# llsurreal919/Reduce-Complexity-for-intra-coding-of-VVC

Measured on AMD Instinct MI355X. Metric: CTUs/sec (All-Intra, QP32), higher is better.
Workload: dtype int16/int32 samples+coefficients, fp64 RD cost

## Files before the change

reduce-complexity-for-intra-coding-of-vvc_amd/csrc/vvcx_dev.h:

```cpp
#pragma once
#include <stdint.h>

#ifndef VXD_NW
#define VXD_NW 4
#endif
#define VXD_NT (VXD_NW * 64)
#ifndef VXD_BUF
#define VXD_BUF 256
#endif
#ifndef VXD_WPE
#define VXD_WPE 5
#endif
#define VXD_MAXD 12
#define VXD_NUM_CTX 291

struct VxUnit {
  uint64_t ss;
  int16_t  x, y;
  uint8_t  lw, lh;
  uint8_t  qt, mt, bt, depth;
  uint8_t  dir, mrl, cbf, mts;
  uint16_t tag;
};

// ... 154 lines not shown
#define VXD_OFF_SLOTS   ((VXD_OFF_CTX + (VXD_MAXD + VXD_NW + 1) * 2 * VXD_CTXSNAP + 255) & ~255)
#define VXD_SLOT_ELEMS  (2 * 4096)
#define VXD_OFF_TMP     (VXD_OFF_SLOTS + VXD_NW * 2 * VXD_SLOT_ELEMS * 2)
struct VxCacheEnt { uint64_t ss; uint8_t kind , dir, mrl, cbf, depth, mts; uint16_t gen ; };
#define VXD_CACHE_ENTRIES (32 * 32 * 5 * 5)
#define VXD_CACHE_DIM   1152
#define VXD_OFF_ORG     (VXD_OFF_TMP + VXD_NW * 2048 * 4)
#define VXD_OFF_LM      (VXD_OFF_ORG + 4096 * 2)
#define VXD_DQ_WAVE     8192
#define VXD_OFF_DQ      ((VXD_OFF_LM + (1024 + 128) * 2 + 255) & ~255)
#define VXD_POOL_ELEMS      32768
#define VXD_POOL_NODE_BYTES (128 * 1024)
#define VXD_POOL_ITEMS      64
struct VxRbItem { double cost; uint64_t dist, bits; int32_t cbf, sum0, test, wave; };
#define VXD_OFF_POOL    ((VXD_OFF_DQ + VXD_NW * VXD_DQ_WAVE + 255) & ~255)
#define VXD_OFF_POOL_COEF  (VXD_OFF_POOL + VXD_POOL_ELEMS * 2)
#define VXD_OFF_POOL_NODES (VXD_OFF_POOL_COEF + VXD_POOL_ELEMS * 2)
#define VXD_OFF_POOL_REC   (VXD_OFF_POOL_NODES + VXD_POOL_NODE_BYTES)
#define VXD_ISP_WAVE    14336
#define VXD_OFF_ISP     ((VXD_OFF_POOL_REC + 2 * VXD_POOL_ITEMS * (int) sizeof(VxRbItem) + 255) & ~255)
#define VXD_OFF_ISP_BEST (VXD_OFF_ISP + VXD_NW * VXD_ISP_WAVE * 2)
#define VXD_OFF_JCCR    ((VXD_OFF_ISP_BEST + 2 * 4096 * 2 + 255) & ~255)
#define VXD_JCCR_WAVE   (6 * 1024 * 2)
#define VXD_OFF_CACHE   ((VXD_OFF_JCCR + VXD_NW * VXD_JCCR_WAVE + 255) & ~255)
#define VXD_OFF_CACHE_LEV (VXD_OFF_CACHE + VXD_CACHE_ENTRIES * (int) sizeof(VxCacheEnt))
#define VXD_OFF_META    (VXD_OFF_CACHE_LEV + VXD_CACHE_DIM * VXD_CACHE_DIM * 2)
#define VXD_SCRATCH_BYTES (VXD_OFF_META + 256)
```

reduce-complexity-for-intra-coding-of-vvc_amd/csrc/vvcx_kernel.hip:

```cpp
#include <hip/hip_runtime.h>
#include <stdint.h>
#define VX_QUAL static __device__ const
#include "vvcx_tables.h"
#include "vvcx_ctu_syntax_tables.h"
#include "vvcx_dev.h"
#include "vvcx_mip_dev.h"

#define NT VXD_NT
#if (VXD_NW & (VXD_NW - 1)) == 0
#define VTX ((threadIdx.x + ((((unsigned) blockIdx.x * 0x9E3779B1u) >> 30) << 6)) & (unsigned) (VXD_NT - 1))
#else
__device__ inline unsigned vtx_rotated()
{
  const unsigned t = threadIdx.x + ((((unsigned) blockIdx.x * 0x9E3779B1u) >> 24) % VXD_NW << 6);
  return t >= VXD_NT ? t - VXD_NT : t;
}
#define VTX (vtx_rotated())
#endif
#define NW VXD_NW
#define MAXD VXD_MAXD
#define BUF VXD_BUF
#define NCTX VXD_NUM_CTX
static_assert(VXD_NUM_CTX == VX_NUM_CTX, "vvcx_dev.h and the generated tables disagree on the number of context models");
#define MAX_DOUBLE 1.7e+308
// ... 69 lines not shown
  int8_t testIsp, ispSlot, ispPrev, ispNT, ispBestMode, ispBestSplit, ispNOrig, ispNList, ispRegN, ispHadN, skipMts2, ispBreak, ispStop[2], ispNumTotal[2], ispCandIdx[2], ispNTested[2];
  uint8_t ispTMode[16], ispTInfo[16], ispList[28], ispReg[16], ispHad[24], ispWinMode, ispWinSplit, ispWinTucbf;
  double ispTCost[16], ispBestRd, ispCurBest, noIspCost;
  unsigned long long ispWinDist, ispWinBits;
  alignas(4) int8_t ispPartsOf[2][68]; int8_t ispFirst[2][2];
  uint8_t inv0[16], rdSrc[24];
};

#define BIN_FRAC(st_, bin_) L.t.bin_frac[(unsigned) (st_) ^ ((0u - (unsigned) (bin_)) & 255u)]
struct Tables {
  uint32_t bin_frac[256];
  int32_t  qscale[12], iqscale[12];
  int16_t  ang[32], inv_ang[32];
  int8_t   gauss[128], cubic[128];
  uint8_t  last_prefix[8], mode_shift[8];
  uint8_t  ctx_rate[NCTX + 2], gorice_pars[32], gorice_pos0[96], rice_len[128], group_idx[64], mode_num[36], intra_thr[8];
  uint8_t  cg_scan[84], grp_scan[228];
  uint8_t  cg_inv[84], grp_inv[228];
};

#define DQ_ABS_SINGLE 64
#define RC_LIST 320
#define DQ_TAB_INTS (21 * 6 + 3 * 12 * 2 + 4)
struct WaveRc { uint16_t binbuf[RC_LIST]; uint8_t binsort[RC_LIST + 8]; };
struct alignas(16) WaveScratch { WaveRc rc; };
struct WaveMem {
  WaveScratch ws;
  alignas(16) int32_t tmp[BUF];
  alignas(16) int16_t slot[2 * BUF];
};
#define CI_CUR 0
#define CI_W(w) (1 + (w))
struct Lds {
  Tables t;
  Ctx ctxs[1 + NW];
  alignas(16) int16_t org[BUF];
  alignas(16) WaveMem wm[NW];
  int acc[NW][4][2];
  int16_t refs[4][2][140];
  uint8_t flags[72]; int8_t src_unit[72];
  int cache_gen, cur_stream;
  int dq_abs[DQ_ABS_SINGLE + NW];
  Frame fr[MAXD];
  int op, op_a, op_b, op_c, op_d, op_ch;
  int pre_copy_d;
  int nx, ny, nw, nh, nd;
  Cand cand[64]; union { double cand_cost[64]; IspRes isp_res[NW]; }; int n_cand;
// ... 429 lines not shown
  rc_serial<WR>(cb, coeff, w, h, is_chroma, scan, pre, zo);
}
__device__ inline int lane_prefix(unsigned long long m)
{
  return (int) __builtin_amdgcn_mbcnt_hi((unsigned) (m >> 32), __builtin_amdgcn_mbcnt_lo((unsigned) m, 0u));
}
__device__ inline int prefix3(int v, int &total)
{
  const unsigned long long b0 = __ballot(v & 1), b1 = __ballot(v & 2), b2 = __ballot(v & 4);
  total = __popcll(b0) + 2 * __popcll(b1) + 4 * __popcll(b2);
  return lane_prefix(b0) + 2 * lane_prefix(b1) + 4 * lane_prefix(b2);
}
__device__ inline int rem_abs_len(unsigned bins, unsigned rice)
{
  const unsigned thr = 5u << rice;
  if (bins < thr) return (int) ((bins >> rice) + 1 + rice);
  const unsigned maxPrefix = 32 - 5 - 15;
  unsigned prefix = 0, suffix, code = (bins >> rice) - 5;
  if (code >= ((1u << maxPrefix) - 1)) { prefix = maxPrefix; suffix = 15; }
  else { while (code > ((2u << prefix) - 2)) prefix++; suffix = prefix + rice + 1; }
  return (int) (5 + prefix + suffix);
}
#define RC_MAXJ 5
__device__ __noinline__ void rc_chain(int ci, int wv, int nb, int lane, unsigned long long &bits)
{
  nb = uni(nb); ci = uni(ci); wv = uni(wv);
  Ctx *c = &L.ctxs[ci]; const uint16_t *bb = L.wm[wv].ws.rc.binbuf; uint8_t *sorted = L.wm[wv].ws.rc.binsort;
  int ctxv[RC_MAXJ]; unsigned binv[RC_MAXJ]; unsigned long long rem[RC_MAXJ];
#pragma unroll
  for (int j = 0; j < RC_MAXJ; j++) {
    const int k = lane + 64 * j;
    const unsigned e = (j * 64 < nb && k < nb) ? bb[k] : 0xffffu;
    ctxv[j] = e == 0xffffu ? -1 : (int) (e >> 1); binv[j] = e & 1;
    rem[j] = j * 64 < nb ? __ballot(ctxv[j] >= 0) : 0ull;
  }
  int segpos = 0;
  for (;;) {
    int nseg = 0, myctx = 0, mystart = 0, mylen = 0;
    for (;;) {
      int v = -1;
#pragma unroll
      for (int j = 0; j < RC_MAXJ; j++) if (v < 0 && rem[j]) v = __builtin_amdgcn_readlane(ctxv[j], __ffsll(rem[j]) - 1);
      if (v < 0) break;
      const int start = segpos;
#pragma unroll
      for (int j = 0; j < RC_MAXJ; j++) if (rem[j]) {
        const unsigned long long m = __ballot(ctxv[j] == v);
        if (ctxv[j] == v) sorted[segpos + lane_prefix(m)] = (uint8_t) binv[j];
        segpos += __popcll(m); rem[j] &= ~m;
      }
      if (lane == nseg) { myctx = v; mystart = start; mylen = segpos - start; }
      if (++nseg == 64) break;
    }
    if (nseg == 0) break;
    wave_sync();
    if (lane < nseg) {
      unsigned a = c->s0[myctx], b = c->s1[myctx];
      const int rate = L.t.ctx_rate[myctx];
      const int r0 = 2 + ((rate >> 2) & 3), r1 = 3 + r0 + (rate & 3);
      const unsigned i0 = (0x7fffu >> r0) & 0x7FE0u, i1 = (0x7fffu >> r1) & 0x7FFEu;
      unsigned acc = 0, pend = 0, nxt = sorted[mystart];
      for (int k = 0; k < mylen; k++) {
        const unsigned bin = nxt;
        nxt = sorted[mystart + k + 1];
        acc += pend;
        pend = BIN_FRAC((a + b) >> 8, bin);
        a -= (a >> r0) & 0x7FE0u; b -= (b >> r1) & 0x7FFEu;
        if (bin) { a += i0; b += i1; }
      }
      c->s0[myctx] = (uint16_t) a; c->s1[myctx] = (uint16_t) b;
      bits += acc + pend;
    }
    wave_sync();
    if (nseg < 64) break;
  }
}
template <bool SMALL>
__device__ __noinline__ void residual_coding_wave(Cab &cb, int lev_off, const int16_t *coeff_g, int w, int h, int is_chroma, int lane, int zo = 0)
{
  coeff_g = uni_p(coeff_g); lev_off = uni(lev_off);
  zo = uni(zo);
  const int dq = uni((int) (L.par.tools & TOOL_DEPQUANT)) != 0;
  int dqx = 0, dqy = 0;
  const long long q0 = STAMP();
  const int16_t *coeff = SMALL ? L.wm[uni(VTX >> 6)].slot + BUF + uni(lev_off) : coeff_g;
  const RcPre pre = rc_prepass_wave<SMALL>(lev_off, coeff_g, w, h, lane);
  const int last = uni(pre.last);
  if (lane == 0) L.rc_last[uni(VTX >> 6)] = last;
  if (last < 0) return;
  w = uni(w); h = uni(h); is_chroma = uni(is_chroma);
  const ScanGeo geo = scan_geo(w, h);
  const long long q1 = STAMP();
  long long qe = 0, qc = 0;
  const int wv = uni(VTX >> 6);
  uint16_t *bb = L.wm[wv].ws.rc.binbuf; uint8_t *sorted = L.wm[wv].ws.rc.binsort;
  const int lcg = geo.lcg, cgSize = 1 << lcg;
  const int zw = imin(32, w), zh = imin(32, h), wg = geo.wg, hg = geo.hg;
  const unsigned long long sigGroups = pre.sig_groups, sigRaster = pre.sig_raster;
  unsigned long long mybits = 0;
  int nb;
  {
    const int l2w = ilog2i(w), l2h = ilog2i(h);
    int offx = 0, offy = 0, shx, shy;
    if (is_chroma) { shx = imin(2, w >> 3); shy = imin(2, h >> 3); }
    else { offx = L.t.last_prefix[l2w]; offy = L.t.last_prefix[l2h]; shx = (l2w + 1) >> 2; shy = (l2h + 1) >> 2; }
    const int blk = scan_blk(geo, last);
    const int posY = blk >> ilog2i(w), posX = blk & (w - 1);
    const int gx = uni(L.t.group_idx[posX]), gy = uni(L.t.group_idx[posY]);
    const int maxX = L.t.group_idx[((zo && w == 32) ? 16 : zw) - 1], maxY = L.t.group_idx[((zo && h == 32) ? 16 : zh) - 1];
    const int nX = gx + (gx < maxX), nY = gy + (gy < maxY);
    if (lane < nX) bb[lane] = (uint16_t) (((VX_CTX_LastX[is_chroma] + offx + (lane >> shx)) << 1) | (lane < gx));
    if (lane < nY) bb[nX + lane] = (uint16_t) (((VX_CTX_LastY[is_chroma] + offy + (lane >> shy)) << 1) | (lane < gy));
    if (lane == 0) mybits += (unsigned long long) ((gx > 3 ? (gx - 2) >> 1 : 0) + (gy > 3 ? (gy - 2) >> 1 : 0)) << 15;
    nb = nX + nY;
  }
  const int sigBase = VX_CTX_SigFlag[is_chroma], g1Base = VX_CTX_GtxFlag[is_chroma + 2], g2Base = VX_CTX_GtxFlag[is_chroma], parBase = VX_CTX_ParFlag[is_chroma];
  const int grpBase = VX_CTX_SigCoeffGroup[is_chroma];
  int regBins = (((zo && w == 32) ? 16 : zw) * ((zo && h == 32) ? 16 : zh) * 28) >> 4;
// ... 56 lines not shown
      const int sigLower = (cgY + 1) < hg ? (int) ((sigRaster >> (cgPos + wg)) & 1) : 0;
      bb[o++] = (uint16_t) (((grpBase + (sigRight | sigLower)) << 1) | (int) ((sigGroups >> sub) & 1));
    }
    int ep = (coded && a) ? 1 : 0;
    if (ctxMode) {
      if (sigCoded) bb[o++] = (uint16_t) (((VX_CTX_SigFlag[is_chroma + 2 * imax(0, qstate - 1)] + sigofs) << 1) | (a != 0));
      if (a) {
        bb[o++] = (uint16_t) (((g1Base + goff) << 1) | (a > 1));
        if (a > 1) {
          bb[o++] = (uint16_t) (((parBase + goff) << 1) | ((a - 2) & 1));
          bb[o++] = (uint16_t) (((g2Base + goff) << 1) | (((a - 2) >> 1) != 0));
          if (a >= 4) ep += rem_abs_len((unsigned) (a - 4) >> 1, L.t.gorice_pars[imax(imin(sumPlain - 20, 31), 0)]);
        }
      }
    } else if (coded) {
      const int sumAll = imin(sumPlain, 31);
      const unsigned rice = L.t.gorice_pars[sumAll], pos0 = L.t.gorice_pos0[imax(0, qstate - 1) * 32 + sumAll];
      ep += rem_abs_len(a == 0 ? pos0 : (unsigned) a <= pos0 ? (unsigned) a - 1 : (unsigned) a, rice);
    }
    mybits += (unsigned long long) ep << 15;
    regBins -= used; nb += tot;
    wave_sync();
    const long long e1 = STAMP();
    rc_chain(cb.ci, wv, nb, lane, mybits);
    nb = 0;
    qe += e1 - e0; qc += STAMP() - e1;
  }
  const long long q3 = STAMP();
  const unsigned long long tot = wave_sum_u64(mybits);
  if (lane == 0) cb.bits += tot;
  if (VVCX_STAMP && VTX == 0) { PROF(32) += (unsigned long long) (q1 - q0); PROF(34) += (unsigned long long) qe; PROF(35) += (unsigned long long) qc; PROF(36) += (unsigned long long) (STAMP() - q3); PROF(37) += 1; }
}

#include "vvcx_depquant_dev.h"
#include "vvcx_lfnst_dev.h"

__device__ int implicit_split(const VxParams &p, Frame &f, int ch)
{
  if (f.impl_checked) return f.impl_split;
  int split = SPLIT_NONE;
  const int blIn = f.x < p.pic_w && (f.y + f.h - 1) < p.pic_h;
  const int trIn = (f.x + f.w - 1) < p.pic_w && f.y < p.pic_h;
  const int maxBt = p.max_bt_size[ch], minQt = p.min_qt[ch];
  const int btAllowed = f.w <= maxBt && f.h <= maxBt;
  const int qtAllowed = f.w > minQt && f.h > minQt && f.bt == 0;
  if (!blIn && !trIn && qtAllowed) split = SPLIT_QT;
  else if (!blIn && btAllowed) split = SPLIT_BH;
// ... 1352 lines not shown
    }
    if (uni(cbf)) residual_coding_wave<SMALL>(cb, 0, lev, w, h, 0, lane, mts > 1);
    if (lane == 0) cost = rd_cost(p, cb.bits, sse);
    if (VVCX_STAMP && VTX == 0) { const long long tb3 = STAMP(); PROF(28) += (unsigned long long) (tb1 - tb0); PROF(29) += (unsigned long long) (tb2 - tb1); PROF(31) += (unsigned long long) (tb3 - tb2); }
    cost = lane0_d(cost);
    if (cost < mbest) {
      mbest = cost;
      if (lane == 0) { L.rd_cost[c] = cost; L.rd_dist[c] = sse; L.rd_bits[c] = cb.bits; L.rd_cbf[c] = (uint8_t) cbf; L.rd_mts[c] = (uint8_t) mts; L.rd_wave[c] = (uint8_t) wave; }
    }
    if (cost < wbest) {
      wbest = cost;
      if (lane == 0) { L.wave_best[wave] = c; L.wave_slot[wave] = SMALL ? 1 : cur; }
      if (SMALL) { int16_t *pr = slot_rec(scratch, P, wave, 1), *pl = slot_lev(scratch, P, wave, 1); for (int i = lane; i < P; i += 64) { pr[i] = rec[i]; pl[i] = lev[i]; } }
      else cur ^= 1;
      { uint32_t *d = (uint32_t *) ctx_ptr(scratch, CTX_START, MAXD + wave, 0); const uint32_t *s = (const uint32_t *) &L.ctxs[CI_W(wave)]; for (int i = lane; i < NCTX; i += 64) d[i] = s[i]; }
    }
    wave_sync();
    }
  }
  if (lane == 0) L.mts_evals[wave] = nmts;
}
template <bool SMALL> __device__ __noinline__ void stage_b_loop_dct2(uint8_t *scratch, int wave, int lane, int w, int h) { stage_b_loop<SMALL, false>(L.par, scratch, wave, lane, w, h); }
template <bool SMALL> __device__ __noinline__ void stage_b_loop_mts(const VxParams &p_, uint8_t *scratch, int wave, int lane, int w, int h) { stage_b_loop<SMALL, true>(L.par, scratch, wave, lane, w, h); (void) p_; }
template <bool SMALL>
__device__ void dq_trellis_phase(uint8_t *scratch, int n, int P, int total, int w, int h, int zo, int wave, int lane, int lfnst = 0, int item0 = 0, int abs0 = 0, int wave_shift = 0)
{
  int16_t *poolCoef = (int16_t *) (scratch + VXD_OFF_POOL_COEF) + (size_t) item0 * P; uint8_t *poolNodes = scratch + VXD_OFF_POOL_NODES + (size_t) item0 * 4 * total;
  const int ipw = imin(16, (int) sizeof(WaveMem) / (240 + 2 * total));
  for (int i0 = ((wave + NW - wave_shift) % NW) * ipw; i0 < n; i0 += NW * ipw)
    wave_depquant_batch<2>(imin(ipw, n - i0), poolCoef + (size_t) i0 * P, P, poolNodes + (size_t) i0 * 4 * total, 4 * total, wave, abs0 + i0,
                        CI_CUR, 0, VX_CTX_QtCbf[0], 0u, w, h, 0, zo, lfnst, lane);
}
template <bool SMALL>
__device__ __noinline__ void stage_b_rounds(uint8_t *scratch, int wave, int lane, int w, int h)
{
  scratch = uni_p(scratch); wave = uni(wave); w = uni(w); h = uni(h);
  const VxParams &p = L.par;
  const int P = w * h, bd = uni(p.bit_depth), total = imin(32, w) * imin(32, h);
  const int mtsOk = mts_allowed(p, w, h);
  const int lfOn = uni((int) (p.tools & TOOL_LFNST)) != 0, psLf = lfOn ? uni((int) L.ps_lfnst) : 0, psMts = lfOn ? uni((int) L.ps_mts) : 0, psGrp = uni((int) L.ps_grp);
  const int pruneOk = mtsOk && !lfOn;
  const int tsOn = lfOn && !psLf && !psMts && ts_allowed(p, w, h);
  int16_t *poolPred = (int16_t *) (scratch + VXD_OFF_POOL), *poolCoef = (int16_t *) (scratch + VXD_OFF_POOL_COEF);
  VxRbItem *recA = (VxRbItem *) (scratch + VXD_OFF_POOL_REC), *recB = recA + VXD_POOL_ITEMS;
  const int capItems = imin(VXD_POOL_ITEMS, imin(VXD_POOL_ELEMS / P, VXD_POOL_NODE_BYTES / (4 * total)));
  const int capCand = imin(16, pruneOk ? imax(1, capItems / 3) : capItems);
// ... 24 lines not shown
        for (int e = lane; e < P; e += 64) { const int py = e >> ilog2i(w), px = e & (w - 1); rec[e] = (int16_t) pred_sample(top, left, w, h, px, py, ip, mode, 1, bd, dcv); }
      }
      wave_sync();
      for (int e = lane; e < P; e += 64) poolPred[(size_t) i * P + e] = rec[e];
      unsigned long long sse; int cbf, sum0 = 0;
      const int mtsC = psMts ? pass_mts_idx(psGrp, mode) : 0;
      if (mtsC) wave_code_block_mts<SMALL>(org, rec, lev, wave_tmp(scratch, imin(w, 32) * h, wave), w, h, bd, p.qp_tr, mtsC, lane, sse, cbf, -2);
      else wave_code_block<SMALL, true>(org, 0, 0, rec, lev, wave_tmp(scratch, imin(w, 32) * h, wave), w, h, bd, p.qp_tr, lane, sse, cbf, -2, &sum0, 0, 0, 0, psLf, psLf ? lfnst_mode(mip ? PLANAR : mode, w, h) : 0);
      for (int e = lane; e < P; e += 64) poolCoef[(size_t) i * P + e] = lev[e];
      if (lane == 0) { recA[i].sum0 = sum0; recA[i].test = 0; recB[i].sum0 = sum0; }
      if (specGen) {
        wave_code_block_mts<SMALL>(org, rec, lev, wave_tmp(scratch, imin(w, 32) * h, wave), w, h, bd, p.qp_tr, 2, lane, sse, cbf, -2);
        for (int e = lane; e < P; e += 64) poolCoef[(size_t) (nA + i) * P + e] = lev[e];
      }
      if (specGen2) {
        wave_code_block<SMALL>(org, 0, 0, rec, lev, wave_tmp(scratch, imin(w, 32) * h, wave), w, h, bd, p.qp_tr, lane, sse, cbf, -2, nullptr, 0, 0, 0, 2, lfnst_mode(mip ? PLANAR : mode, w, h));
        for (int e = lane; e < P; e += 64) poolCoef[(size_t) (nA + i) * P + e] = lev[e];
      }
    }
    __threadfence_block();
    __syncthreads();
    const long long q1 = STAMP();
    if (!specUse) dq_trellis_phase<SMALL>(scratch, nA, P, total, w, h, psMts, wave, lane, psLf);
    if (specGen) dq_trellis_phase<SMALL>(scratch, nA, P, total, w, h, 1, wave, lane, 0, nA, 32, 1);
    if (specGen2) dq_trellis_phase<SMALL>(scratch, nA, P, total, w, h, 0, wave, lane, 2, nA, 32, 1);
    if (tsEarly && wave >= 2) {
      for (int i = wave - 2; i < nA; i += 2) {
        const int sa = wave_ts_fwd(org, poolPred + (size_t) i * P, poolCoef + (size_t) (48 + i) * P, w, h, bd, lane);
        if (lane == 0) L.rb_pairs[i] = (uint8_t) ((double) sa <= (double) recB[i].sum0);
      }
      __threadfence_block();
      wave_sync();
      int cnt = 0, mine = -1;
      for (int i = wave - 2; i < nA; i += 2) if (L.rb_pairs[i]) { if (cnt == lane) mine = i; cnt++; }
      if (mine >= 0) L.dq_abs[48 + mine] = ts_rdoq_lane(poolCoef + (size_t) (48 + mine) * P, w, h, bd, p.qp_tr);
    }
    __threadfence_block();
    __syncthreads();
    const long long q2 = STAMP();
    if (specGen || specGen2) { if ((int) VTX < nA) L.spec_abs[VTX] = L.dq_abs[32 + VTX]; if (VTX == 0) { L.spec_n = (int8_t) nA; L.spec_kind = (int8_t) (specGen ? 1 : 2); } }
    else if (VTX == 0) L.spec_n = 0;
    for (int i = wave; i < nA; i += NW) {
      const int c = c0 + i, mode = uni(L.rd[c].mode), mrl = uni(L.rd[c].mrl);
      int16_t *rec = SMALL ? L.wm[wave].slot : slot_rec(scratch, P, wave, cur), *lev = SMALL ? L.wm[wave].slot + BUF : slot_lev(scratch, P, wave, cur);
      const int mtsC = psMts ? pass_mts_idx(psGrp, mode) : 0;
      const int src = specUse ? (specKind == 2 ? i : uni((int) L.rd_src[c])) : i;
      for (int e = lane; e < P; e += 64) { rec[e] = poolPred[(size_t) src * P + e]; lev[e] = poolCoef[(size_t) (specUse ? specN + src : i) * P + e]; }
      wave_sync();
// ... 125 lines not shown
        { uint32_t *d = (uint32_t *) &L.ctxs[CI_W(wave)]; const uint32_t *s = (const uint32_t *) &L.ctxs[CI_CUR]; for (int e = lane; e < NCTX; e += 64) d[e] = s[e]; }
        wave_sync();
        double cost = 0;
        Cab cb; cb.ci = CI_W(wave); cb.bits = 0;
        if (lane == 0) { enc_intra_luma_pred_mode(cb, L.ny, mode, mrl); enc_bin(cb, 1u, VX_CTX_QtCbf[0]); enc_tu_mts(cb, w, h, mts); }
        residual_coding_wave<SMALL>(cb, 0, lev, w, h, 0, lane, 1);
        if (lane == 0) { cost = rd_cost(p, cb.bits, sse); recB[j].cost = cost; recB[j].dist = sse; recB[j].bits = cb.bits; }
        cost = lane0_d(cost);
        if (cost < wbest || (cost == wbest && c * 8 + k < wkey)) {
          wbest = cost; wkey = c * 8 + k;
          if (lane == 0) { L.wave_best[wave] = c; L.wave_slot[wave] = SMALL ? 1 : cur; }
          if (SMALL) { int16_t *pr = slot_rec(scratch, P, wave, 1), *pl = slot_lev(scratch, P, wave, 1); for (int e = lane; e < P; e += 64) { pr[e] = rec[e]; pl[e] = lev[e]; } }
          else cur ^= 1;
          { uint32_t *d = (uint32_t *) ctx_ptr(scratch, CTX_START, MAXD + wave, 0); const uint32_t *s = (const uint32_t *) &L.ctxs[CI_W(wave)]; for (int e = lane; e < NCTX; e += 64) d[e] = s[e]; }
        }
        wave_sync();
      }
      __threadfence_block();
      __syncthreads();
    }
    if (VVCX_STAMP && VTX == 0) { PROF(38) += (unsigned long long) (q1 - q0); PROF(39) += (unsigned long long) (q2 - q1); PROF(40) += (unsigned long long) (q3 - q2); PROF(41) += (unsigned long long) (STAMP() - q3); PROF(44) += 1; PROF(45) += (unsigned long long) nA; }
#ifdef VVCX_STAMP_PASS
    if (VTX == 0) { const int kind = psMts ? 3 + psGrp : psLf; PROF(16 + kind) += 1; PROF(23 + kind) += (unsigned long long) (q2 - q1); }
#endif
    if ((int) VTX < nA) {
      const int i = VTX, c = c0 + i;
      double bc = recA[i].cost; uint64_t bd_ = recA[i].dist, bb = recA[i].bits; int bcbf = recA[i].cbf, bm = 0, bw = recA[i].wave;
      for (int j = 0; j < nB; j++) if ((pi_[j] >> 3) == i) { const double v = recB[j].cost; if (v < bc) { bc = v; bd_ = recB[j].dist; bb = recB[j].bits; bcbf = 1; bm = (pi_[j] & 7) + 1; bw = recB[j].wave; } }
      if (lfOn) { bm = recA[i].sum0 >> 8; L.rd_lfl[c] = (uint8_t) (recA[i].sum0 & 3); }
      L.rd_cost[c] = bc; L.rd_dist[c] = bd_; L.rd_bits[c] = bb; L.rd_cbf[c] = (uint8_t) bcbf; L.rd_mts[c] = (uint8_t) bm; L.rd_wave[c] = (uint8_t) bw;
    }
    __syncthreads();
  }
  if (lane == 0) L.mts_evals[wave] = nmts;
}
__device__ __noinline__ void op_stage_b(const VxParams &p_, uint8_t *scratch)
{
  scratch = uni_p(scratch);
  const VxParams &p = L.par; (void) p_;
  const int wave = uni(VTX >> 6), lane = VTX & 63;
  const int w = uni(L.nw), h = uni(L.nh);
  if (uni(p.tools & TOOL_DEPQUANT)) { if (w * h <= BUF) stage_b_rounds<true>(scratch, wave, lane, w, h); else stage_b_rounds<false>(scratch, wave, lane, w, h); }
  else if (uni(p.tools & TOOL_MTS)) { if (w * h <= BUF) stage_b_loop_mts<true>(p, scratch, wave, lane, w, h); else stage_b_loop_mts<false>(p, scratch, wave, lane, w, h); }
  else if (w * h <= BUF) stage_b_loop_dct2<true>(scratch, wave, lane, w, h); else stage_b_loop_dct2<false>(scratch, wave, lane, w, h);
  __threadfence_block();
  __syncthreads();
// ... 115 lines not shown
__device__ inline int ict_mode(int sign, int mask) { const int m = mask == 1 ? 3 : mask == 2 ? 1 : 2; return sign ? -m : m; }
__device__ inline int ict_fwd(int b, int r, int mode, long long &err)
{
  int v, eb, er;
  switch (mode) {
    case  1: v = (4 * b + 2 * r) / 5; eb = b - v; er = r - (v >> 1); break;
    case -1: v = (4 * b - 2 * r) / 5; eb = b - v; er = r - (-v >> 1); break;
    case  2: v = (b + r) / 2; eb = b - v; er = r - v; break;
    case -2: v = (b - r) / 2; eb = b - v; er = r + v; break;
    case  3: v = (4 * r + 2 * b) / 5; eb = b - (v >> 1); er = r - v; break;
    default: v = (4 * r - 2 * b) / 5; eb = b - (-v >> 1); er = r - v; break;
  }
  err += (long long) eb * eb + (long long) er * er;
  return v;
}
__device__ inline int ict_inv(int c, int mode, int k)
{
  const int am = mode < 0 ? -mode : mode, sc = mode < 0 ? -c : c;
  if (am == 3) return k == 1 ? c : (sc >> 1);
  return k == 0 ? c : (am == 1 ? (sc >> 1) : sc);
}
__device__ inline long long wave_sum_i64(long long v) { return (long long) wave_sum_u64((unsigned long long) v); }

template <bool SMALL>
__device__ __noinline__ void chroma_rd_rounds(uint8_t *scratch, int wave, int lane, int w, int h)
{
  scratch = uni_p(scratch); wave = uni(wave); w = uni(w); h = uni(h);
  const VxParams &p = L.par;
  const int P = w * h, bd = uni(p.bit_depth), total = imin(32, w) * imin(32, h);
  const int16_t *lmin = lm_in_buf(scratch, 2 * P);
  const int16_t *org = org_tile(scratch, 2 * P);
  int16_t *poolPred = (int16_t *) (scratch + VXD_OFF_POOL), *poolCoef = (int16_t *) (scratch + VXD_OFF_POOL_COEF); uint8_t *poolNodes = scratch + VXD_OFF_POOL_NODES;
  if (lane == 0) L.wave_best[wave] = -1;
  dq_build_tables(1);
  double wbest = MAX_DOUBLE;
  int cur = 0;
  const int n_rd = uni(L.n_rd);
  const int psLf = (uni((int) (p.tools & TOOL_LFNST)) && w >= 4 && h >= 4) ? uni((int) L.ps_lfnst) : 0;
  const int jccrOn = uni((int) (p.tools & TOOL_JCCR)) != 0;
  const int cadj = P > 4 ? uni(L.lmcs_cadj) : 0;
  int njoint = 0;
#define CHROMA_LFMODE(c_) (psLf ? lfnst_mode((uni((int) L.rd[c_].mode) >= LM_CHROMA && uni((int) L.rd[c_].mode) <= MDLM_T) ? uni(L.colm) : uni((int) L.rd[c_].mrl), w, h) : 0)
  for (int c = wave; c < n_rd; c += NW) {
    const int fm = uni(L.rd[c].mrl), lfm = CHROMA_LFMODE(c);
    int16_t *recb = SMALL ? L.wm[wave].slot : slot_rec(scratch, 2 * P, wave, cur), *levb = SMALL ? L.wm[wave].slot + BUF : slot_lev(scratch, 2 * P, wave, cur);
    for (int k = 0; k < 2; k++) {
// ... 5 lines not shown
      wave_code_block<SMALL>(org, k * P, k * P, rec, lev, wave_tmp(scratch, imin(w, 32) * h, wave), w, h, bd, p.qp_tr_c[k], lane, sse, cbf, -2, nullptr, k + 1, CI_CUR, 0, psLf, lfm, 0, -1, cadj);
      for (int e = lane; e < P; e += 64) poolCoef[(size_t) (2 * c + k) * P + e] = lev[e];
      wave_sync();
    }
  }
  __threadfence_block();
  __syncthreads();
  {
    const int ipw = imin(16, (int) sizeof(WaveMem) / (240 + 2 * total));
    for (int i0 = wave * ipw; i0 < n_rd; i0 += NW * ipw)
      wave_depquant_batch<2>(imin(ipw, n_rd - i0), poolCoef + (size_t) (2 * i0) * P, 2 * P, poolNodes + (size_t) (2 * i0) * 4 * total, 8 * total, wave, i0,
                          CI_CUR, 0, VX_CTX_QtCbf[1], 0u, w, h, 1, 0, psLf, lane);
  }
  __threadfence_block();
  __syncthreads();
  const bool crBatch = 4 * (240 + 2 * total) <= (int) (sizeof(WaveScratch) + sizeof(int32_t) * BUF);
  for (int c0 = 0; c0 < n_rd; c0 += NW) {
    const int c = c0 + wave; const bool have = c < n_rd;
    const int cm = have ? uni(L.rd[c].mode) : 0;
    const int lfm = have ? CHROMA_LFMODE(c) : 0;
    int16_t *recb = SMALL ? L.wm[wave].slot : slot_rec(scratch, 2 * P, wave, cur), *levb = SMALL ? L.wm[wave].slot + BUF : slot_lev(scratch, 2 * P, wave, cur);
    unsigned long long dist = 0; int cbfs[2] = { 0, 0 };
    double compCost = 0; int jccr = 0;
    if (have) {
      { uint32_t *d = (uint32_t *) &L.ctxs[CI_W(wave)]; const uint32_t *s_ = (const uint32_t *) &L.ctxs[CI_CUR]; for (int e = lane; e < NCTX; e += 64) d[e] = s_[e]; }
      for (int e = lane; e < P; e += 64) { recb[e] = poolPred[(size_t) (2 * c) * P + e]; levb[e] = poolCoef[(size_t) (2 * c) * P + e]; }
      wave_sync();
      cbfs[0] = uni(L.dq_abs[c]) > 0;
      unsigned long long sse; int cbf2;
      wave_code_block<SMALL>(org, 0, 0, recb, levb, wave_tmp(scratch, imin(w, 32) * h, wave), w, h, bd, p.qp_tr_c[0], lane, sse, cbf2, cbfs[0], nullptr, 1, CI_W(wave), 0, psLf, lfm, 0, -1, cadj);
      dist += (unsigned long long) (p.dist_weight[0] * (double) sse);
      { Cab cb; cb.ci = CI_W(wave); cb.bits = 0; if (lane == 0) enc_bin(cb, (unsigned) cbfs[0], VX_CTX_QtCbf[1]); if (cbfs[0]) residual_coding_wave<SMALL>(cb, 0, levb, w, h, 1, lane);
        double c0 = 0; if (lane == 0) c0 = rd_cost(p, cb.bits, dist); compCost = lane0_d(c0); }
      wave_sync();
      if (lane == 0) L.rb_pairs[wave] = (uint8_t) cbfs[0];
    }
    __threadfence_block();
    __syncthreads();
    {
      const int n4 = imin(NW, n_rd - c0);
      unsigned mask = 0; for (int i = 0; i < n4; i++) mask |= (unsigned) L.rb_pairs[i] << i;
      if (crBatch) { if (wave == 0) wave_depquant_batch<0>(n4, poolCoef + (size_t) (2 * c0 + 1) * P, 2 * P, poolNodes + (size_t) (2 * c0 + 1) * 4 * total, 8 * total, 0, c0,
                                                        CI_W(0), 1, VX_CTX_QtCbf[2], mask, w, h, 2, 0, psLf, lane); }
      else if (have) wave_depquant_batch<0>(1, poolCoef + (size_t) (2 * c + 1) * P, 0, poolNodes + (size_t) (2 * c + 1) * 4 * total, 0, wave, c,
                                         CI_W(wave), 0, VX_CTX_QtCbf[2], (unsigned) cbfs[0], w, h, 2, 0, psLf, lane);
    }
// ... 42 lines not shown
            long long dm = 0; int b = org[e] - pCb[e], r = org[P + e] - pCr[e];
            if (cadj) { b = lmcs_scale_fwd(b, cadj, bd); r = lmcs_scale_fwd(r, cadj, bd); }
            jres[e] = (int16_t) ict_fwd(b, r, mode, dm); jout[e] = 0;
          }
          wave_sync();
          njoint++;
          unsigned long long sseJ; int cbfJ;
          wave_code_block<false>(jres, 0, 0, jout, jlev, wave_tmp(scratch, imin(w, 32) * h, wave), w, h, bd, mask == 3 ? p.qp_tr_j : p.qp_tr_c[comp - 1], lane, sseJ, cbfJ, -1, nullptr, comp, CI_CUR, 0, psLf, lfm, 1, 2 + mask);
          if (!cbfJ) continue;
          unsigned long long sCb = 0, sCr = 0;
          const int mx = (1 << bd) - 1;
          for (int e = lane; e < P; e += 64) {
            const int cj = jout[e];
            int rb = ict_inv(cj, mode, 0), rr = ict_inv(cj, mode, 1);
            if (cadj) { rb = lmcs_scale_inv((int) (int16_t) rb, cadj, bd); rr = lmcs_scale_inv((int) (int16_t) rr, cadj, bd); }
            int vb = pCb[e] + rb, vr = pCr[e] + rr;
            vb = vb < 0 ? 0 : vb > mx ? mx : vb; vr = vr < 0 ? 0 : vr > mx ? mx : vr;
            jres[e] = (int16_t) vb; jout[e] = (int16_t) vr;
            const int db = org[e] - vb, dr = org[P + e] - vr;
            sCb += (unsigned long long) (db * db); sCr += (unsigned long long) (dr * dr);
          }
          sCb = wave_sum_u64(sCb); sCr = wave_sum_u64(sCr);
          const unsigned long long dJ = (unsigned long long) (p.dist_weight[0] * (double) sCb) + (unsigned long long) (p.dist_weight[1] * (double) sCr);
          { uint32_t *d = (uint32_t *) &L.ctxs[CI_W(wave)]; const uint32_t *s_ = (const uint32_t *) &L.ctxs[CI_CUR]; for (int e = lane; e < NCTX; e += 64) d[e] = s_[e]; }
          wave_sync();
          Cab cb; cb.ci = CI_W(wave); cb.bits = 0;
          if (lane == 0) { enc_bin(cb, (unsigned) (mask >> 1), VX_CTX_QtCbf[1]); enc_bin(cb, (unsigned) (mask & 1), VX_CTX_QtCbf[2] + (mask >> 1)); enc_bin(cb, 1u, VX_CTX_JointCbCrFlag + mask - 1); }
          residual_coding_wave<false>(cb, 0, jlev, w, h, 1, lane);
          double cj = 0; if (lane == 0) cj = rd_cost(p, cb.bits, dJ);
          cj = lane0_d(cj);
          if (cj < compCost) {
            compCost = cj; jccr = mask; bestJDist = dJ;
            for (int e = lane; e < P; e += 64) { brec[e] = jres[e]; brec[P + e] = jout[e]; blev[e] = jlev[e]; }
          }
          wave_sync();
        }
        if (jccr) {
          dist = bestJDist; cbfs[0] = jccr >> 1; cbfs[1] = jccr & 1;
          for (int e = lane; e < P; e += 64) { recb[e] = brec[e]; recb[P + e] = brec[P + e]; levb[e] = (jccr >> 1) ? blev[e] : 0; levb[P + e] = (jccr >> 1) ? 0 : blev[e]; }
        }
        wave_sync();
      }
      if (jccrOn) {
        { uint32_t *d = (uint32_t *) &L.ctxs[CI_W(wave)]; const uint32_t *s_ = (const uint32_t *) &L.ctxs[CI_CUR]; for (int e = lane; e < NCTX; e += 64) d[e] = s_[e]; }
        wave_sync();
        Cab cb; cb.ci = CI_W(wave); cb.bits = 0;
        const int msk = (cbfs[0] ? 2 : 0) | (cbfs[1] ? 1 : 0);
        if (!jccr) {
          if (lane == 0) enc_bin(cb, (unsigned) cbfs[0], VX_CTX_QtCbf[1]);
          if (cbfs[0]) residual_coding_wave<SMALL>(cb, 0, levb, w, h, 1, lane);
          if (lane == 0) { enc_bin(cb, (unsigned) cbfs[1], VX_CTX_QtCbf[2] + cbfs[0]); if (msk) enc_bin(cb, 0u, VX_CTX_JointCbCrFlag + msk - 1); }
          if (cbfs[1]) residual_coding_wave<SMALL>(cb, P, levb + P, w, h, 1, lane);
        } else {
          if (lane == 0) { enc_bin(cb, (unsigned) cbfs[0], VX_CTX_QtCbf[1]); enc_bin(cb, (unsigned) cbfs[1], VX_CTX_QtCbf[2] + cbfs[0]); enc_bin(cb, 1u, VX_CTX_JointCbCrFlag + msk - 1); }
          if (jccr >> 1) residual_coding_wave<SMALL>(cb, 0, levb, w, h, 1, lane); else residual_coding_wave<SMALL>(cb, P, levb + P, w, h, 1, lane);
        }
        wave_sync();
      }
      double cost = 0;
      {
        Cab cb; cb.ci = CI_W(wave); cb.bits = 0;
        if (lane == 0) {
          enc_intra_chroma_pred_mode(cb, cm, L.colm, L.lm_ok);
          enc_bin(cb, (unsigned) cbfs[0], VX_CTX_QtCbf[1]);
          enc_bin(cb, (unsigned) cbfs[1], VX_CTX_QtCbf[2] + cbfs[0]);
          if (jccrOn && (cbfs[0] | cbfs[1])) enc_bin(cb, jccr ? 1u : 0u, VX_CTX_JointCbCrFlag + ((cbfs[0] ? 2 : 0) | (cbfs[1] ? 1 : 0)) - 1);
        }
        int fl = 0;
        if (cbfs[0]) { residual_coding_wave<SMALL>(cb, 0, levb, w, h, 1, lane); fl |= lfnst_flags(uni(L.rc_last[wave]), w, h); }
        if (cbfs[1] && jccr != 3) { residual_coding_wave<SMALL>(cb, P, levb + P, w, h, 1, lane); fl |= lfnst_flags(uni(L.rc_last[wave]), w, h); }
        if (lane == 0) {
          cost = rd_cost(p, cb.bits, dist);
          L.rd_cost[c] = cost; L.rd_dist[c] = dist; L.rd_cbf[c] = (uint8_t) ((cbfs[0] ? 2 : 0) | (cbfs[1] ? 4 : 0)); L.rd_lfl[c] = (uint8_t) fl; L.rd_mts[c] = (uint8_t) jccr;
        }
      }
      cost = lane0_d(cost);
      if (cost < wbest) {
        wbest = cost;
        if (lane == 0) { L.wave_best[wave] = c; L.wave_slot[wave] = SMALL ? 1 : cur; }
        if (SMALL) { int16_t *pr = slot_rec(scratch, 2 * P, wave, 1), *pl = slot_lev(scratch, 2 * P, wave, 1); for (int e = lane; e < 2 * P; e += 64) { pr[e] = recb[e]; pl[e] = levb[e]; } }
        else cur ^= 1;
// ... 881 lines not shown
        L.op_c = f.nmodes > 1;
        return 1;
      }
      return 0;
}

__device__ __noinline__ void ctrl_train_label(const Frame &f, int row)
{
  const VxParams &p = L.par; const VxFrameDev &fd = L.fdv;
  int label = -1;
  if (f.best.cost != MAX_DOUBLE) label = (int) ((fd.units[0][(f.y >> 2) * p.uw + (f.x >> 2)].ss >> (f.depth * 5)) & 31);
  p.train_rows[(size_t) row * 28 + 27] = label;
}
__device__ __attribute__((always_inline)) inline void control_step(const VxParams &p, const VxFrameDev &fd, uint8_t *scratch)
{
  CtlState &S = L.S;
  const int ch = L.tree_ch, tile = L.cur_tile, sh = ch ? 1 : 0;
  for (;;) {
    if (L.d < 0) { post(OP_DONE); return; }
    Frame &f = L.fr[L.d];
    const int d = L.d;
#if VVCX_STAMP
    const long long tph = STAMP(); const int phs = f.phase;
#if !defined(VVCX_STAMP_DQ) && !defined(VVCX_STAMP_ISP) && !defined(VVCX_STAMP_PASS)
    struct PhStamp { long long t; int ph; __device__ ~PhStamp() { const int slot = ph < 12 ? 16 + ph : ph == PH_EXIT2 ? 1 : ph == PH_A3_DONE ? 28 : ph == PH_PASS ? 29 : ph == PH_NEXT_PASS ? 31 : 47; PROF(slot) += (unsigned long long) (STAMP() - t); PROF(30) += 1; } } phstamp = { tph, phs };
#endif
#endif
#ifdef VX_TRACE
    fprintf(stderr, "  step d %d phase %d nmodes %d\n", d, f.phase, f.nmodes);
#endif
    switch (f.phase) {
    case PH_ENTER: {
      L.cnt[3]++;
      init_cu_level(p, fd, scratch, d, ch, tile);
      f.best.cost = MAX_DOUBLE; f.best.dist = 0; f.best.bits = 0; f.best.valid = 0;
      if (f.nmodes == 0) { f.phase = PH_EXIT2; break; }
      f.phase = PH_RUN; f.ctx_dirty = 0;
      L.pre_copy_d = d;
      L.train_row[d] = -1;
      if (((p.tools & TOOL_FAST) || p.train_rows) && !ch && fast_candidates(p, fd, f, tile)) { f.phase = PH_FAST_DONE; set_node(f, d); post(OP_FAST); return; }
      break;
    }
    case PH_FAST_DONE: {
      const int res = L.fa_res;
      L.train_row[d] = L.fa_row;
      if (res >= 0 && res <= 5) {
        const int mode = res == 0 ? ETM_INTRA : res == 1 ? ETM_SPLIT_QT : res == 2 ? ETM_SPLIT_BT_H : res == 3 ? ETM_SPLIT_BT_V : res == 4 ? ETM_SPLIT_TT_H : ETM_SPLIT_TT_V;
// ... 1063 lines not shown
```

Baseline: 185.4.

## Match rate-estimation contexts via ballots and snapshot chroma contexts instead of re-encoding

Replaces the sorted-segment context chain in rate estimation with a ballot-based scheme: lanes holding bins of the same context are found by comparing nine context-id bits across the wave, and one owner lane walks the bins for that context serially. This drops the sort buffer and its passes. Chroma RD now snapshots the wave's context state after the first JCCR trial and after the best trial and restores it, instead of re-running residual coding to rebuild the contexts. It also adds an optional single-list DQ spec-shift knob, off by default, plus profiling stamps. The snapshots need extra per-wave scratch, and the owner loop is serial when many bins share one context.

```diff
diff --git a/reduce-complexity-for-intra-coding-of-vvc_amd/csrc/vvcx_dev.h b/reduce-complexity-for-intra-coding-of-vvc_amd/csrc/vvcx_dev.h
--- a/reduce-complexity-for-intra-coding-of-vvc_amd/csrc/vvcx_dev.h
+++ b/reduce-complexity-for-intra-coding-of-vvc_amd/csrc/vvcx_dev.h
@@ -200,7 +200,8 @@
 #define VXD_OFF_ISP_BEST (VXD_OFF_ISP + VXD_NW * VXD_ISP_WAVE * 2)
 #define VXD_OFF_JCCR    ((VXD_OFF_ISP_BEST + 2 * 4096 * 2 + 255) & ~255)
 #define VXD_JCCR_WAVE   (6 * 1024 * 2)
-#define VXD_OFF_CACHE   ((VXD_OFF_JCCR + VXD_NW * VXD_JCCR_WAVE + 255) & ~255)
+#define VXD_OFF_JCTX    ((VXD_OFF_JCCR + VXD_NW * VXD_JCCR_WAVE + 255) & ~255)
+#define VXD_OFF_CACHE   ((VXD_OFF_JCTX + VXD_NW * 2 * VXD_CTXSNAP + 255) & ~255)
 #define VXD_OFF_CACHE_LEV (VXD_OFF_CACHE + VXD_CACHE_ENTRIES * (int) sizeof(VxCacheEnt))
 #define VXD_OFF_META    (VXD_OFF_CACHE_LEV + VXD_CACHE_DIM * VXD_CACHE_DIM * 2)
 #define VXD_SCRATCH_BYTES (VXD_OFF_META + 256)
diff --git a/reduce-complexity-for-intra-coding-of-vvc_amd/csrc/vvcx_kernel.hip b/reduce-complexity-for-intra-coding-of-vvc_amd/csrc/vvcx_kernel.hip
--- a/reduce-complexity-for-intra-coding-of-vvc_amd/csrc/vvcx_kernel.hip
+++ b/reduce-complexity-for-intra-coding-of-vvc_amd/csrc/vvcx_kernel.hip
@@ -115,7 +115,14 @@
 #define DQ_ABS_SINGLE 64
 #define RC_LIST 320
 #define DQ_TAB_INTS (21 * 6 + 3 * 12 * 2 + 4)
+#ifndef VXD_RC_MATCH
+#define VXD_RC_MATCH 1
+#endif
+#if VXD_RC_MATCH
+struct WaveRc { uint16_t binbuf[RC_LIST]; uint8_t trellis_room[RC_LIST + 8]; };
+#else
 struct WaveRc { uint16_t binbuf[RC_LIST]; uint8_t binsort[RC_LIST + 8]; };
+#endif
 struct alignas(16) WaveScratch { WaveRc rc; };
 struct WaveMem {
   WaveScratch ws;
@@ -591,10 +598,66 @@
   return (int) (5 + prefix + suffix);
 }
 #define RC_MAXJ 5
+#if VXD_RC_MATCH
+static_assert(NCTX <= 512, "rc_chain matches context ids on nine bits");
+__device__ __noinline__ unsigned rc_chain(int ci, int wv, int nb, int lane)
+{
+  nb = uni(nb); ci = uni(ci); wv = uni(wv);
+  Ctx *c = &L.ctxs[ci]; const uint16_t *bb = L.wm[wv].ws.rc.binbuf;
+  unsigned bits = 0;
+#ifdef VVCX_STAMP_RC
+  int st_ctx = 0;
+#endif
+  for (int base = 0; base < nb; base += 64) {
+    const bool valid = base + lane < nb;
+    const unsigned e = valid ? bb[base + lane] : 0u;
+    const unsigned ctx = e >> 1;
+    unsigned long long same = __ballot(valid);
+#pragma unroll
+    for (int b = 0; b < 9; b++) {
+      const unsigned long long m = __ballot((ctx >> b) & 1);
+      same &= ((ctx >> b) & 1) ? m : ~m;
+    }
+    const unsigned long long binm = __ballot(e & 1);
+    const unsigned blo = (unsigned) binm, bhi = (unsigned) (binm >> 32);
+    const bool owner = valid && lane_prefix(same) == 0;
+#ifdef VVCX_STAMP_RC
+    st_ctx += __popcll(__ballot(owner));
+#endif
+    if (owner) {
+      unsigned a = c->s0[ctx], b = c->s1[ctx];
+      const int rate = L.t.ctx_rate[ctx];
+      const int r0 = 2 + ((rate >> 2) & 3), r1 = 3 + r0 + (rate & 3);
+      const unsigned i0 = (0x7fffu >> r0) & 0x7FE0u, i1 = (0x7fffu >> r1) & 0x7FFEu;
+      unsigned mlo = (unsigned) same, mhi = (unsigned) (same >> 32), acc = 0, pend = 0;
+      do {
+        const bool lo = mlo != 0;
+        const unsigned mm = lo ? mlo : mhi, low = mm & (0u - mm);
+        const unsigned bin = ((lo ? blo : bhi) & low) != 0;
+        if (lo) mlo ^= low; else mhi ^= low;
+        acc += pend;
+        pend = BIN_FRAC((a + b) >> 8, bin);
+        a -= (a >> r0) & 0x7FE0u; b -= (b >> r1) & 0x7FFEu;
+        if (bin) { a += i0; b += i1; }
+      } while (mlo | mhi);
+      c->s0[ctx] = (uint16_t) a; c->s1[ctx] = (uint16_t) b;
+      bits += acc + pend;
+    }
+    wave_sync();
+  }
+#ifdef VVCX_STAMP_RC
+  if (VTX == 0) { PROF(16) += 1; PROF(17) += (unsigned long long) nb; PROF(18) += (unsigned long long) st_ctx; if ((unsigned long long) nb > PROF(19)) PROF(19) = (unsigned long long) nb; if ((unsigned long long) st_ctx > PROF(20)) PROF(20) = (unsigned long long) st_ctx; }
+#endif
+  return bits;
+}
+#else
 __device__ __noinline__ void rc_chain(int ci, int wv, int nb, int lane, unsigned long long &bits)
 {
   nb = uni(nb); ci = uni(ci); wv = uni(wv);
   Ctx *c = &L.ctxs[ci]; const uint16_t *bb = L.wm[wv].ws.rc.binbuf; uint8_t *sorted = L.wm[wv].ws.rc.binsort;
+#ifdef VVCX_STAMP_RC
+  int st_ctx = 0;
+#endif
   int ctxv[RC_MAXJ]; unsigned binv[RC_MAXJ]; unsigned long long rem[RC_MAXJ];
 #pragma unroll
   for (int j = 0; j < RC_MAXJ; j++) {
@@ -622,6 +685,9 @@
       if (++nseg == 64) break;
     }
     if (nseg == 0) break;
+#ifdef VVCX_STAMP_RC
+    st_ctx += nseg;
+#endif
     wave_sync();
     if (lane < nseg) {
       unsigned a = c->s0[myctx], b = c->s1[myctx];
@@ -643,7 +709,11 @@
     wave_sync();
     if (nseg < 64) break;
   }
-}
+#ifdef VVCX_STAMP_RC
+  if (VTX == 0) { PROF(16) += 1; PROF(17) += (unsigned long long) nb; PROF(18) += (unsigned long long) st_ctx; if ((unsigned long long) nb > PROF(19)) PROF(19) = (unsigned long long) nb; if ((unsigned long long) st_ctx > PROF(20)) PROF(20) = (unsigned long long) st_ctx; }
+#endif
+}
+#endif
 template <bool SMALL>
 __device__ __noinline__ void residual_coding_wave(Cab &cb, int lev_off, const int16_t *coeff_g, int w, int h, int is_chroma, int lane, int zo = 0)
 {
@@ -662,7 +732,7 @@
   const long long q1 = STAMP();
   long long qe = 0, qc = 0;
   const int wv = uni(VTX >> 6);
-  uint16_t *bb = L.wm[wv].ws.rc.binbuf; uint8_t *sorted = L.wm[wv].ws.rc.binsort;
+  uint16_t *bb = L.wm[wv].ws.rc.binbuf;
   const int lcg = geo.lcg, cgSize = 1 << lcg;
   const int zw = imin(32, w), zh = imin(32, h), wg = geo.wg, hg = geo.hg;
   const unsigned long long sigGroups = pre.sig_groups, sigRaster = pre.sig_raster;
@@ -765,7 +835,11 @@
     regBins -= used; nb += tot;
     wave_sync();
     const long long e1 = STAMP();
+#if VXD_RC_MATCH
+    mybits += rc_chain(cb.ci, wv, nb, lane);
+#else
     rc_chain(cb.ci, wv, nb, lane, mybits);
+#endif
     nb = 0;
     qe += e1 - e0; qc += STAMP() - e1;
   }
@@ -2164,6 +2238,9 @@
 }
 template <bool SMALL> __device__ __noinline__ void stage_b_loop_dct2(uint8_t *scratch, int wave, int lane, int w, int h) { stage_b_loop<SMALL, false>(L.par, scratch, wave, lane, w, h); }
 template <bool SMALL> __device__ __noinline__ void stage_b_loop_mts(const VxParams &p_, uint8_t *scratch, int wave, int lane, int w, int h) { stage_b_loop<SMALL, true>(L.par, scratch, wave, lane, w, h); (void) p_; }
+#ifndef VXD_DQ_ONE_LIST
+#define VXD_DQ_ONE_LIST 0
+#endif
 template <bool SMALL>
 __device__ void dq_trellis_phase(uint8_t *scratch, int n, int P, int total, int w, int h, int zo, int wave, int lane, int lfnst = 0, int item0 = 0, int abs0 = 0, int wave_shift = 0)
 {
@@ -2234,8 +2311,9 @@
     __syncthreads();
     const long long q1 = STAMP();
     if (!specUse) dq_trellis_phase<SMALL>(scratch, nA, P, total, w, h, psMts, wave, lane, psLf);
-    if (specGen) dq_trellis_phase<SMALL>(scratch, nA, P, total, w, h, 1, wave, lane, 0, nA, 32, 1);
-    if (specGen2) dq_trellis_phase<SMALL>(scratch, nA, P, total, w, h, 0, wave, lane, 2, nA, 32, 1);
+    const int ipwB = imin(16, (int) sizeof(WaveMem) / (240 + 2 * total)), specShift = VXD_DQ_ONE_LIST ? ((nA + ipwB - 1) / ipwB) % NW : 1;
+    if (specGen) dq_trellis_phase<SMALL>(scratch, nA, P, total, w, h, 1, wave, lane, 0, nA, 32, specShift);
+    if (specGen2) dq_trellis_phase<SMALL>(scratch, nA, P, total, w, h, 0, wave, lane, 2, nA, 32, specShift);
     if (tsEarly && wave >= 2) {
       for (int i = wave - 2; i < nA; i += 2) {
         const int sa = wave_ts_fwd(org, poolPred + (size_t) i * P, poolCoef + (size_t) (48 + i) * P, w, h, bd, lane);
@@ -2407,6 +2485,13 @@
     if (VVCX_STAMP && VTX == 0) { PROF(38) += (unsigned long long) (q1 - q0); PROF(39) += (unsigned long long) (q2 - q1); PROF(40) += (unsigned long long) (q3 - q2); PROF(41) += (unsigned long long) (STAMP() - q3); PROF(44) += 1; PROF(45) += (unsigned long long) nA; }
 #ifdef VVCX_STAMP_PASS
     if (VTX == 0) { const int kind = psMts ? 3 + psGrp : psLf; PROF(16 + kind) += 1; PROF(23 + kind) += (unsigned long long) (q2 - q1); }
+    if (VTX == 0 && !psMts && psLf == 0) {
+      const int ipw_ = imin(16, (int) sizeof(WaveMem) / (240 + 2 * total)), nch = (nA + ipw_ - 1) / ipw_;
+      const int n1 = specUse ? 0 : nch, n2 = (specGen || specGen2) ? nch : 0;
+      int worst = 0;
+      for (int wv = 0; wv < NW; wv++) { int k = 0; for (int i = 0; i < n1; i++) k += i % NW == wv; for (int i = 0; i < n2; i++) k += (i + (VXD_DQ_ONE_LIST ? n1 : 1)) % NW == wv; worst = imax(worst, k); }
+      if (worst >= 2) { PROF(30) += 1; PROF(47) += (unsigned long long) (q2 - q1); if (n1 + n2 <= NW) PROF(33) += (unsigned long long) (q2 - q1); }
+    }
 #endif
     if ((int) VTX < nA) {
       const int i = VTX, c = c0 + i;
@@ -2568,6 +2653,9 @@
 }
 __device__ inline long long wave_sum_i64(long long v) { return (long long) wave_sum_u64((unsigned long long) v); }
 
+#ifndef VXD_CHROMA_CTX_SNAP
+#define VXD_CHROMA_CTX_SNAP 1
+#endif
 template <bool SMALL>
 __device__ __noinline__ void chroma_rd_rounds(uint8_t *scratch, int wave, int lane, int w, int h)
 {
@@ -2619,6 +2707,10 @@
     int16_t *recb = SMALL ? L.wm[wave].slot : slot_rec(scratch, 2 * P, wave, cur), *levb = SMALL ? L.wm[wave].slot + BUF : slot_lev(scratch, 2 * P, wave, cur);
     unsigned long long dist = 0; int cbfs[2] = { 0, 0 };
     double compCost = 0; int jccr = 0;
+#if VXD_CHROMA_CTX_SNAP
+    uint32_t *snap = (uint32_t *) (scratch + VXD_OFF_JCTX + (size_t) wave * 2 * VXD_CTXSNAP);
+    int snapped = 0;
+#endif
     if (have) {
       { uint32_t *d = (uint32_t *) &L.ctxs[CI_W(wave)]; const uint32_t *s_ = (const uint32_t *) &L.ctxs[CI_CUR]; for (int e = lane; e < NCTX; e += 64) d[e] = s_[e]; }
       for (int e = lane; e < P; e += 64) { recb[e] = poolPred[(size_t) (2 * c) * P + e]; levb[e] = poolCoef[(size_t) (2 * c) * P + e]; }
@@ -2707,6 +2799,9 @@
           }
           sCb = wave_sum_u64(sCb); sCr = wave_sum_u64(sCr);
           const unsigned long long dJ = (unsigned long long) (p.dist_weight[0] * (double) sCb) + (unsigned long long) (p.dist_weight[1] * (double) sCr);
+#if VXD_CHROMA_CTX_SNAP
+          if (!snapped) { const uint32_t *s_ = (const uint32_t *) &L.ctxs[CI_W(wave)]; for (int e = lane; e < NCTX; e += 64) snap[e] = s_[e]; snapped = 1; }
+#endif
           { uint32_t *d = (uint32_t *) &L.ctxs[CI_W(wave)]; const uint32_t *s_ = (const uint32_t *) &L.ctxs[CI_CUR]; for (int e = lane; e < NCTX; e += 64) d[e] = s_[e]; }
           wave_sync();
           Cab cb; cb.ci = CI_W(wave); cb.bits = 0;
@@ -2717,6 +2812,9 @@
           if (cj < compCost) {
             compCost = cj; jccr = mask; bestJDist = dJ;
             for (int e = lane; e < P; e += 64) { brec[e] = jres[e]; brec[P + e] = jout[e]; blev[e] = jlev[e]; }
+#if VXD_CHROMA_CTX_SNAP
+            { const uint32_t *s_ = (const uint32_t *) &L.ctxs[CI_W(wave)]; for (int e = lane; e < NCTX; e += 64) snap[NCTX + e] = s_[e]; }
+#endif
           }
           wave_sync();
         }
@@ -2726,6 +2824,13 @@
         }
         wave_sync();
       }
+#if VXD_CHROMA_CTX_SNAP
+      if (snapped) {
+        const uint32_t *s_ = snap + (jccr ? NCTX : 0); uint32_t *d = (uint32_t *) &L.ctxs[CI_W(wave)];
+        for (int e = lane; e < NCTX; e += 64) d[e] = s_[e];
+        wave_sync();
+      }
+#else
       if (jccrOn) {
         { uint32_t *d = (uint32_t *) &L.ctxs[CI_W(wave)]; const uint32_t *s_ = (const uint32_t *) &L.ctxs[CI_CUR]; for (int e = lane; e < NCTX; e += 64) d[e] = s_[e]; }
         wave_sync();
@@ -2742,6 +2847,7 @@
         }
         wave_sync();
       }
+#endif
       double cost = 0;
       {
         Cab cb; cb.ci = CI_W(wave); cb.bits = 0;
@@ -3669,7 +3775,7 @@
     const int d = L.d;
 #if VVCX_STAMP
     const long long tph = STAMP(); const int phs = f.phase;
-#if !defined(VVCX_STAMP_DQ) && !defined(VVCX_STAMP_ISP) && !defined(VVCX_STAMP_PASS)
+#if !defined(VVCX_STAMP_DQ) && !defined(VVCX_STAMP_ISP) && !defined(VVCX_STAMP_PASS) && !defined(VVCX_STAMP_RC)
     struct PhStamp { long long t; int ph; __device__ ~PhStamp() { const int slot = ph < 12 ? 16 + ph : ph == PH_EXIT2 ? 1 : ph == PH_A3_DONE ? 28 : ph == PH_PASS ? 29 : ph == PH_NEXT_PASS ? 31 : 47; PROF(slot) += (unsigned long long) (STAMP() - t); PROF(30) += 1; } } phstamp = { tph, phs };
 #endif
 #endif
```

New measurement: 192.7, median of 6. +4.0%, better.
